# blindopen/TSM-Det-Pointcloud-

Measured on AMD Instinct MI355X. Metric: point-cloud frames/sec (fwd+bwd), higher is better.
Workload: dtype f32; 1 GPU; BASELINE configs[1]: KITTI-shaped synthetic, 20000 pts / 16000 active voxels per frame, full SECOND detector (VoxelBackBone8x) fwd+bwd+AdamW step; batch_per_gpu=4, global_batch=4, parallelism=dp1, voxelize_on_gpu=True

## Files before the change

tsm-det-pointcloud-_amd/csrc/conv_wgrad.hip:

```cpp
#include "spx_common.h"

#ifdef SPX_WG_DIAG
__device__ unsigned long long* g_wg_diag = nullptr;
extern "C" int spx_diag_set(unsigned long long* p) { return (int)hipMemcpyToSymbol(HIP_SYMBOL(g_wg_diag), &p, sizeof(p)); }
#define DIAG_T() __builtin_amdgcn_s_memtime()
#endif

namespace {

typedef float f32x4 __attribute__((ext_vector_type(4)));

#ifndef SPX_SB
#define SPX_SB __builtin_amdgcn_sched_barrier(0)
#endif
constexpr int kGroups = 4;
#ifndef SPX_WG_BURST
#define SPX_WG_BURST 4
#endif
constexpr int kBurst = SPX_WG_BURST;

static inline int wgrad_splits(int64_t n, int cin, int cout, int kvol) {
  int64_t s = n / (64 * kGroups);
  constexpr int slab_mb = 32;
  int64_t by_slab = (int64_t(slab_mb) << 20) / ((int64_t)kvol * cin * cout * 4);
  if (s > by_slab) s = by_slab;
  constexpr int max_blocks = 2048;
  int64_t by_blocks = max_blocks / kvol;
  if (by_blocks < 8) by_blocks = 8;
  if (s > by_blocks) s = by_blocks;
  if (s < 1) s = 1;
  return (int)s;
}

__device__ __forceinline__ void wgrad_plan(const int32_t* __restrict__ cnt, int K, int J, int lane, int& sk, int& start,
                                           int& mycnt) {
  const uint32_t cval = lane < K ? (uint32_t)cnt[lane] : 0u;
  mycnt = (int)cval;
  uint64_t total = cval;
#pragma unroll
  for (int o = 32; o > 0; o >>= 1) total += __shfl_xor(total, o);
  int sh = 0;
  while ((total >> sh) >= (1u << 19)) ++sh;
  const uint32_t tot_s = (uint32_t)(total >> sh);
  sk = 0;
  if (lane < K) sk = tot_s > 0 ? 1 + (int)(((uint32_t)(J - K) * (cval >> sh)) / tot_s) : J / K;
  int incl = sk;
#pragma unroll
  for (int o = 1; o < 64; o <<= 1) {
    int t = __shfl_up(incl, o);
    if (lane >= o) incl += t;
  }
  start = incl - sk;
}

constexpr int kCntUnroll = 4;
__global__ __launch_bounds__(1024) void k_wgrad_count(const int32_t* __restrict__ pair, int64_t ld, int64_t n,
                                                      const int64_t* d_n, int K, int G, int32_t* __restrict__ cnt64,
                                                      int32_t* __restrict__ cnt8) {
  __shared__ int32_t part[16];
  const int x = blockIdx.x, k = blockIdx.y;
  const int lane = threadIdx.x & 63, w = threadIdx.x >> 6;
  const int64_t nlive = spx_live_n(d_n, n);
  const int64_t n8 = ((nlive + 7) / 8 + 63) / 64 * 64;
  const int64_t g0 = x * (n8 / 64);
  int64_t g1 = g0 + n8 / 64;
  const int64_t glive = (nlive + 63) / 64;
  if (g1 > glive) g1 = glive;
  const int32_t* prow = pair + (int64_t)k * ld;
  int total = 0;
  for (int64_t g = g0 + w * kCntUnroll; g < g1; g += 16 * kCntUnroll) {
    int32_t id[kCntUnroll];
#pragma unroll
    for (int u = 0; u < kCntUnroll; ++u) {
      const int64_t row = 64 * (g + u) + lane;
      id[u] = (g + u < g1 && row < nlive) ? prow[row] : -1;
    }
#pragma unroll
    for (int u = 0; u < kCntUnroll; ++u) {
      const int c = __popcll(__ballot(id[u] >= 0));
      if (lane == 0 && g + u < g1) cnt64[(size_t)k * G + g + u] = c;
      total += c;
    }
  }
  if (lane == 0) part[w] = total;
  __syncthreads();
  if (threadIdx.x == 0) {
    int t = 0;
#pragma unroll
    for (int i = 0; i < 16; ++i) t += part[i];
    cnt8[x * 32 + k] = t;
  }
}

template <int W>
__device__ __forceinline__ void load_vec(const float* __restrict__ p, float (&v)[W]) {
  if constexpr (W == 1) {
    v[0] = p[0];
  } else if constexpr (W == 2) {
    float2 t = *reinterpret_cast<const float2*>(p);
    v[0] = t.x, v[1] = t.y;
  } else {
#pragma unroll
    for (int i = 0; i < W; i += 4) {
      float4 t = *reinterpret_cast<const float4*>(p + i);
      v[i] = t.x, v[i + 1] = t.y, v[i + 2] = t.z, v[i + 3] = t.w;
    }
  }
}

template <int W>
__device__ __forceinline__ void store_vec(float* __restrict__ p, const float (&v)[W]) {
  if constexpr (W == 1) {
    p[0] = v[0];
  } else if constexpr (W == 2) {
    *reinterpret_cast<float2*>(p) = make_float2(v[0], v[1]);
  } else {
#pragma unroll
    for (int i = 0; i < W; i += 4) *reinterpret_cast<float4*>(p + i) = make_float4(v[i], v[i + 1], v[i + 2], v[i + 3]);
  }
}

template <int MI, int NJ, bool EXACT, bool FULL>
__device__ __forceinline__ void wgrad_fetch(const float* __restrict__ in, int cin, const float* __restrict__ dout,
                                            int cout, const int32_t* q_src, const int32_t* q_dst, int p, int npairs,
                                            int c, float (&a)[MI], float (&b)[NJ]) {
  const bool has = FULL || (p < npairs);
  const int32_t sid = has ? q_src[p] : 0;
  const int32_t did = has ? q_dst[p] : 0;
  if (EXACT && FULL) {
    load_vec<MI>(in + (size_t)sid * cin + MI * c, a);
    load_vec<NJ>(dout + (size_t)did * cout + NJ * c, b);
  } else {
#pragma unroll
    for (int mi = 0; mi < MI; ++mi) {
      int ci = MI * c + mi;
      a[mi] = (has && ci < cin) ? in[(size_t)sid * cin + ci] : 0.f;
    }
#pragma unroll
    for (int nj = 0; nj < NJ; ++nj) {
      int co = NJ * c + nj;
      b[nj] = (has && co < cout) ? dout[(size_t)did * cout + co] : 0.f;
    }
  }
}

template <int MI, int NJ>
__device__ __forceinline__ void wgrad_mfma_step(f32x4 (&acc)[MI][NJ], const float (&a)[MI], const float (&b)[NJ]) {
#pragma unroll
  for (int mi = 0; mi < MI; ++mi)
#pragma unroll
    for (int nj = 0; nj < NJ; ++nj) acc[mi][nj] = __builtin_amdgcn_mfma_f32_16x16x4f32(a[mi], b[nj], acc[mi][nj], 0, 0, 0);
}

template <int MI, int NJ, bool EXACT>
__global__ __launch_bounds__(64) void k_wgrad_mfma(const float* __restrict__ in, int cin,
                                                   const float* __restrict__ dout, int cout,
                                                   const int32_t* __restrict__ pair, int64_t ld, int64_t n,
                                                   const int64_t* d_n, const int32_t* __restrict__ cnt64,
                                                   const int32_t* __restrict__ cnt8, int G, int J, int K,
                                                   float* __restrict__ slab) {
  __shared__ int32_t q_src[64 * kGroups + 4];
  __shared__ int32_t q_dst[64 * kGroups + 4];
  const int lane = threadIdx.x;
  const int c = lane & 15, q = lane >> 4;
  const int xcd = blockIdx.x & 7, j = blockIdx.x >> 3;
  int sk, start, mycnt;
  wgrad_plan(cnt8 + xcd * 32, K, J, lane, sk, start, mycnt);
  const unsigned long long mine = __ballot(lane < K && j >= start && j < start + sk);
  if (mine == 0) return;
  const int k = __ffsll((long long)mine) - 1;
  const int sub = __builtin_amdgcn_readfirstlane(j - __shfl(start, k));
  const int nsub = __builtin_amdgcn_readfirstlane(__shfl(sk, k));
  const int64_t total = __builtin_amdgcn_readfirstlane(__shfl(mycnt, k));
  const int64_t nlive = spx_live_n(d_n, n);
  const int64_t n8 = ((nlive + 7) / 8 + 63) / 64 * 64;
  const int64_t lo = total * sub / nsub, hi = total * (sub + 1) / nsub;
  const int gx0 = (int)(xcd * (n8 / 64));
  int gx1 = gx0 + (int)(n8 / 64);
  const int glive = (int)((nlive + 63) / 64);
  if (gx1 > glive) gx1 = glive;
  int n_lo = 0, n_hi = 0;
  int64_t run = 0;
  for (int g = gx0; g < gx1; g += 64) {
    const int v = g + lane < gx1 ? cnt64[(size_t)k * G + g + lane] : 0;
    int incl = v;
#pragma unroll
    for (int o = 1; o < 64; o <<= 1) {
      int t = __shfl_up(incl, o);
      if (lane >= o) incl += t;
    }
    const int64_t excl = run + incl - v;
    const bool in = g + lane < gx1;
    n_lo += __popcll(__ballot(in && excl < lo));
    n_hi += __popcll(__ballot(in && excl < hi));
    run += __shfl(incl, 63);
  }
  int64_t r0 = 64 * (int64_t)(gx0 + n_lo);
  int64_t r1 = 64 * (int64_t)(gx0 + n_hi);
  if (r1 > nlive) r1 = nlive;
  if (r0 > r1) r0 = r1;

#ifdef SPX_WG_DIAG
  const unsigned long long d_t0 = DIAG_T(), d_r0 = __builtin_amdgcn_s_memrealtime();
  unsigned long long d_steps = 0, d_loop = 0, d_nsteps = 0;
#endif
  f32x4 acc[MI][NJ];
#pragma unroll
  for (int mi = 0; mi < MI; ++mi)
#pragma unroll
    for (int nj = 0; nj < NJ; ++nj) acc[mi][nj] = f32x4{0.f, 0.f, 0.f, 0.f};

  const int32_t* prow = pair + (int64_t)k * ld;
  int carry = 0;
  int32_t idn[kGroups];
  const int64_t rlast = r1 > r0 ? r1 - 1 : 0;
#pragma unroll
  for (int g = 0; g < kGroups; ++g) {
    int64_t row = r0 + 64 * g + lane;
    idn[g] = prow[row < rlast ? row : rlast];
  }
  for (int64_t base = r0; base < r1; base += 64 * kGroups) {
    int32_t id[kGroups];
#pragma unroll
    for (int g = 0; g < kGroups; ++g) {
      id[g] = base + 64 * g + lane < r1 ? idn[g] : -1;
      int64_t row = base + 64 * (kGroups + g) + lane;
      idn[g] = prow[row < rlast ? row : rlast];
    }
    int nvalid = carry;
#pragma unroll
    for (int g = 0; g < kGroups; ++g) {
      unsigned long long mask = __ballot(id[g] >= 0);
      int rank = nvalid + __builtin_amdgcn_mbcnt_hi((unsigned)(mask >> 32), __builtin_amdgcn_mbcnt_lo((unsigned)mask, 0u));
      if (id[g] >= 0) {
        q_src[rank] = id[g];
        q_dst[rank] = (int32_t)(base + 64 * g + lane);
      }
      nvalid += __popcll(mask);
    }
    const int full = nvalid >> 2;
    carry = nvalid & 3;
    if (full == 0) continue;
    __builtin_amdgcn_wave_barrier();
    const int last = full - 1;
#ifdef SPX_WG_DIAG
    const unsigned long long d_a = DIAG_T();
    d_nsteps += full;
#endif
    for (int st = 0; st < full; st += kBurst) {
      float a[kBurst][MI], b[kBurst][NJ];
#pragma unroll
      for (int g = 0; g < kBurst; ++g) {
        const int sg = st + g < last ? st + g : last;
        wgrad_fetch<MI, NJ, EXACT, true>(in, cin, dout, cout, q_src, q_dst, 4 * sg + q, 4, c, a[g], b[g]);
      }
      asm volatile("" ::: "memory");
      __builtin_amdgcn_sched_barrier(0);
#pragma unroll
      for (int g = 0; g < kBurst; ++g) {
        if (g > 0) {
          const float keep = st + g < full ? 1.f : 0.f;
#pragma unroll
          for (int nj = 0; nj < NJ; ++nj) b[g][nj] *= keep;
        }
        wgrad_mfma_step<MI, NJ>(acc, a[g], b[g]);
      }
    }
#ifdef SPX_WG_DIAG
    d_loop += DIAG_T() - d_a;
#endif
    __builtin_amdgcn_wave_barrier();
    if (carry) {
      int32_t ts = 0, td = 0;
      if (lane < carry) ts = q_src[4 * full + lane], td = q_dst[4 * full + lane];
      __builtin_amdgcn_wave_barrier();
      if (lane < carry) q_src[lane] = ts, q_dst[lane] = td;
    }
    __builtin_amdgcn_wave_barrier();
  }
  int ntail = carry ? 1 : 0;
  ntail = __builtin_amdgcn_readfirstlane(ntail);
  asm volatile("" : "+s"(ntail));
  for (int t = 0; t < ntail; ++t) {
    __builtin_amdgcn_wave_barrier();
    float a0[MI], b0[NJ];
    wgrad_fetch<MI, NJ, EXACT, false>(in, cin, dout, cout, q_src, q_dst, q, carry, c, a0, b0);
    wgrad_mfma_step<MI, NJ>(acc, a0, b0);
  }

#ifdef SPX_WG_DIAG
  if (g_wg_diag && lane == 0) {
    unsigned long long* o = g_wg_diag + (size_t)blockIdx.x * 8;
    const unsigned long long t1 = DIAG_T();
    o[0] = t1 - d_t0;
    o[1] = d_loop;
    o[2] = d_nsteps;
    o[3] = __builtin_amdgcn_s_memrealtime() - d_r0;
    o[4] = k;
    o[5] = d_t0;
    o[6] = t1;
    o[7] = (unsigned long long)(r1 > r0 ? r1 - r0 : 0);
  }
#endif
  float* out = slab + ((size_t)xcd * J + j) * cin * cout;
#pragma unroll
  for (int mi = 0; mi < MI; ++mi)
#pragma unroll
    for (int e = 0; e < 4; ++e) {
      const int ci = MI * (4 * q + e) + mi;
      if (EXACT) {
        float v[NJ];
#pragma unroll
        for (int nj = 0; nj < NJ; ++nj) v[nj] = acc[mi][nj][e];
        store_vec<NJ>(out + (size_t)ci * cout + NJ * c, v);
      } else if (ci < cin) {
#pragma unroll
        for (int nj = 0; nj < NJ; ++nj) {
          int co = NJ * c + nj;
          if (co < cout) out[(size_t)ci * cout + co] = acc[mi][nj][e];
        }
      }
    }
}

constexpr int kRedSlices = 16;
__global__ __launch_bounds__(64 * kRedSlices) void k_wgrad_reduce(const float* __restrict__ slab,
                                                                   const int32_t* __restrict__ cnt8, int J, int K, int cin,
                                                                   int cout, float* __restrict__ dw) {
  __shared__ float part[kRedSlices][64];
  __shared__ int p_off[9][32], p_start[8][32];
  {
    const int w = threadIdx.x >> 6, lane = threadIdx.x & 63;
    if (w < 8) {
      int sk, start, mycnt;
      wgrad_plan(cnt8 + w * 32, K, J, lane, sk, start, mycnt);
      if (lane < 32) p_off[w + 1][lane] = sk, p_start[w][lane] = start;
    }
  }
  __syncthreads();
  if (threadIdx.x < 32) {
    int run = 0;
    for (int x = 0; x < 8; ++x) {
      int v = p_off[x + 1][threadIdx.x];
      p_off[x][threadIdx.x] = run;
      run += v;
    }
    p_off[8][threadIdx.x] = run;
  }
  __syncthreads();
  const int per = cin * cout;
  const int total = K * per;
  const int e = threadIdx.x & 63, sl = threadIdx.x >> 6;
  const int t = blockIdx.x * 64 + e;
  float acc4[4] = {0.f, 0.f, 0.f, 0.f};
  if (t < total) {
    const int k = t / per, el = t - k * per;
    const int len = p_off[8][k];
    int x = 0;
    for (int i = sl; i < len; i += 4 * kRedSlices) {
#pragma unroll
      for (int u = 0; u < 4; ++u) {
        const int ii = i + u * kRedSlices;
        if (ii < len) {
          while (ii >= p_off[x + 1][k]) ++x;
          acc4[u] += slab[((size_t)x * J + p_start[x][k] + (ii - p_off[x][k])) * per + el];
        }
      }
    }
  }
  part[sl][e] = (acc4[0] + acc4[1]) + (acc4[2] + acc4[3]);
  __syncthreads();
  if (sl == 0 && t < total) {
    float v = 0.f;
#pragma unroll
    for (int i = 0; i < kRedSlices; ++i) v += part[i][e];
    int co = t % cout, ci = (t / cout) % cin, k = t / per;
    dw[((size_t)co * K + k) * cin + ci] = v;
  }
}

}

static inline int wgrad_blocks_per_xcd(int64_t n, int cin, int cout, int kvol) {
  int J = (wgrad_splits(n, cin, cout, kvol) * kvol + 7) / 8;
  return J < kvol ? kvol : J;
}

static inline size_t wgrad_slab_bytes(int cin, int cout, int kvol, int64_t n) {
  return spx_align((size_t)8 * wgrad_blocks_per_xcd(n, cin, cout, kvol) * cin * cout * sizeof(float));
}
static inline size_t wgrad_cnt64_bytes(int kvol, int64_t n) {
  return spx_align((size_t)kvol * (size_t)((n + 63) / 64 + 1) * sizeof(int32_t));
}

extern "C" size_t spx_conv_wgrad_ws_bytes(int cin, int cout, int kvol, int64_t n_out) {
  return wgrad_slab_bytes(cin, cout, kvol, n_out) + wgrad_cnt64_bytes(kvol, n_out) + spx_align(8 * 32 * sizeof(int32_t));
}

#define SPX_WG_CASE(A, B)                                                                                          \
  if (MI == A && NJ == B) {                                                                                        \
    if (exact)                                                                                                     \
      hipLaunchKernelGGL((k_wgrad_mfma<A, B, true>), dim3(8 * J), dim3(64), 0, s, in, cin, dout, cout, pair, pair_ld, n_out, \
                         d_n_out, cnt64, cnt8, G, J, kvol, slab);                                                  \
    else                                                                                                           \
      hipLaunchKernelGGL((k_wgrad_mfma<A, B, false>), dim3(8 * J), dim3(64), 0, s, in, cin, dout, cout, pair, pair_ld, n_out, \
                         d_n_out, cnt64, cnt8, G, J, kvol, slab);                                                  \
    launched = true;                                                                                               \
  }

extern "C" size_t spx_conv_wgrad_counts_bytes(int kvol, int64_t n_out) {
  return wgrad_cnt64_bytes(kvol, n_out < 0 ? 0 : n_out) + spx_align(8 * 32 * sizeof(int32_t));
}

extern "C" int spx_conv_wgrad_counts(const int32_t* pair, int64_t pair_ld, int kvol, int64_t n_out, const int64_t* d_n_out,
                                     int32_t* counts, spx_stream_t stream) {
  if (!pair || !counts || kvol <= 0 || kvol > SPX_MAX_KVOL || n_out <= 0 || pair_ld < n_out) return SPX_ERR_INVALID_ARG;
  if (n_out >= (int64_t(1) << 31)) return SPX_ERR_TOO_LARGE;
  const int G = (int)((n_out + 63) / 64 + 1);
  int32_t* cnt8 = reinterpret_cast<int32_t*>(reinterpret_cast<char*>(counts) + wgrad_cnt64_bytes(kvol, n_out));
  hipLaunchKernelGGL(k_wgrad_count, dim3(8, kvol), dim3(1024), 0, spx_s(stream), pair, pair_ld, n_out, d_n_out, kvol, G,
                     counts, cnt8);
  SPX_CHECK_LAUNCH();
  return SPX_OK;
}

extern "C" int spx_conv_wgrad(const float* in, int cin, const float* dout, int cout, int kvol, const int32_t* pair,
                              int64_t pair_ld, int64_t n_out, const int64_t* d_n_out, const int32_t* counts, float* dw,
                              void* ws, size_t ws_bytes, spx_stream_t stream) {
  if (!in || !dout || !pair || !dw || cin <= 0 || cout <= 0 || kvol <= 0 || kvol > SPX_MAX_KVOL || n_out < 0 ||
      pair_ld < n_out)
    return SPX_ERR_INVALID_ARG;
  if (cin > 128 || cout > 128) return SPX_ERR_UNSUPPORTED;
  if (n_out >= (int64_t(1) << 31)) return SPX_ERR_TOO_LARGE;
  if (!ws || ws_bytes < spx_conv_wgrad_ws_bytes(cin, cout, kvol, n_out)) return SPX_ERR_WORKSPACE;
  hipStream_t s = spx_s(stream);
  if (n_out == 0) {
    spx_fill_async(dw, 0, sizeof(float) * (size_t)cout * kvol * cin, s);
    return SPX_OK;
  }
  const int J = wgrad_blocks_per_xcd(n_out, cin, cout, kvol);
  const int G = (int)((n_out + 63) / 64 + 1);
  const int32_t* cnt64 = counts;
  const int32_t* cnt8 = counts ? reinterpret_cast<const int32_t*>(reinterpret_cast<const char*>(counts) + wgrad_cnt64_bytes(kvol, n_out))
                               : nullptr;
  if (!counts) {
    int32_t* c64 = reinterpret_cast<int32_t*>(reinterpret_cast<char*>(ws) + wgrad_slab_bytes(cin, cout, kvol, n_out));
    int32_t* c8 = reinterpret_cast<int32_t*>(reinterpret_cast<char*>(c64) + wgrad_cnt64_bytes(kvol, n_out));
    hipLaunchKernelGGL(k_wgrad_count, dim3(8, kvol), dim3(1024), 0, s, pair, pair_ld, n_out, d_n_out, kvol, G, c64, c8);
    cnt64 = c64;
    cnt8 = c8;
  }
  float* slab = reinterpret_cast<float*>(ws);
  int MI = (cin + 15) / 16, NJ = (cout + 15) / 16;
  if (MI == 3) MI = 4;
  if (MI > 4) MI = 8;
  if (NJ == 3) NJ = 4;
  if (NJ > 4) NJ = 8;
  bool launched = false;
  const bool exact = cin == 16 * MI && cout == 16 * NJ;
  SPX_WG_CASE(1, 1)
  SPX_WG_CASE(1, 2)
  SPX_WG_CASE(1, 4)
  SPX_WG_CASE(1, 8)
  SPX_WG_CASE(2, 1)
  SPX_WG_CASE(2, 2)
  SPX_WG_CASE(2, 4)
  SPX_WG_CASE(2, 8)
  SPX_WG_CASE(4, 1)
  SPX_WG_CASE(4, 2)
  SPX_WG_CASE(4, 4)
  SPX_WG_CASE(4, 8)
  SPX_WG_CASE(8, 1)
  SPX_WG_CASE(8, 2)
  SPX_WG_CASE(8, 4)
  SPX_WG_CASE(8, 8)
  if (!launched) return SPX_ERR_UNSUPPORTED;
  int total = kvol * cin * cout;
  hipLaunchKernelGGL(k_wgrad_reduce, dim3((total + 63) / 64), dim3(64 * kRedSlices), 0, s, slab, cnt8, J, kvol, cin, cout, dw);
  SPX_CHECK_LAUNCH();
  return SPX_OK;
}
```

Before: 295.6 frames/s.

## Team four wgrad waves per block and combine partials in LDS before slab write

The sparse-conv weight-gradient kernel now groups four split waves into one 256-thread block. Waves that work on the same kernel offset add their MFMA accumulators through shared memory, so only the leading wave writes a partial tile to the slab. The slab shrinks from one entry per split to one per run, and the reduce kernel changes to fewer slices with run-based indexing and 32-bit addressing. This cuts slab write and read traffic but adds block barriers, more shared memory per block, and idle waves in teams that straddle offsets.

```diff
diff --git a/tsm-det-pointcloud-_amd/csrc/conv_wgrad.hip b/tsm-det-pointcloud-_amd/csrc/conv_wgrad.hip
--- a/tsm-det-pointcloud-_amd/csrc/conv_wgrad.hip
+++ b/tsm-det-pointcloud-_amd/csrc/conv_wgrad.hip
@@ -51,6 +51,19 @@
     if (lane >= o) incl += t;
   }
   start = incl - sk;
+}
+
+constexpr int kTeam = 4;
+__device__ __forceinline__ void wgrad_runs(int sk, int start, int K, int lane, int& nrun, int& rbase) {
+  nrun = lane < K ? ((start + sk - 1) / kTeam) - (start / kTeam) + 1 : 0;
+  const unsigned long long split = __ballot(lane >= 1 && lane < K && (start % kTeam) != 0);
+  rbase = (start + kTeam - 1) / kTeam +
+          (int)__builtin_amdgcn_mbcnt_hi((unsigned)(split >> 32), __builtin_amdgcn_mbcnt_lo((unsigned)split, 0u));
+}
+
+__host__ __device__ static inline int wgrad_runs_per_xcd(int J, int K) {
+  const int r = (J + kTeam - 1) / kTeam + K - 1;
+  return r < J ? r : J;
 }
 
 constexpr int kCntUnroll = 4;
@@ -152,26 +165,47 @@
     for (int nj = 0; nj < NJ; ++nj) acc[mi][nj] = __builtin_amdgcn_mfma_f32_16x16x4f32(a[mi], b[nj], acc[mi][nj], 0, 0, 0);
 }
 
+template <int MI, int NJ>
+struct WgCombine {
+  static constexpr int kTiles = MI * NJ >= 16 ? 8 : MI * NJ >= 8 ? 4 : MI * NJ >= 2 ? 2 : 1;
+  static constexpr int kPasses = MI * NJ / kTiles;
+};
+
 template <int MI, int NJ, bool EXACT>
-__global__ __launch_bounds__(64) void k_wgrad_mfma(const float* __restrict__ in, int cin,
-                                                   const float* __restrict__ dout, int cout,
-                                                   const int32_t* __restrict__ pair, int64_t ld, int64_t n,
-                                                   const int64_t* d_n, const int32_t* __restrict__ cnt64,
-                                                   const int32_t* __restrict__ cnt8, int G, int J, int K,
-                                                   float* __restrict__ slab) {
-  __shared__ int32_t q_src[64 * kGroups + 4];
-  __shared__ int32_t q_dst[64 * kGroups + 4];
-  const int lane = threadIdx.x;
+__global__ __launch_bounds__(64 * kTeam) void k_wgrad_mfma(const float* __restrict__ in, int cin,
+                                                           const float* __restrict__ dout, int cout,
+                                                           const int32_t* __restrict__ pair, int64_t ld, int64_t n,
+                                                           const int64_t* d_n, const int32_t* __restrict__ cnt64,
+                                                           const int32_t* __restrict__ cnt8, int G, int J, int K,
+                                                           float* __restrict__ slab) {
+  constexpr int kTiles = WgCombine<MI, NJ>::kTiles, kPasses = WgCombine<MI, NJ>::kPasses;
+  __shared__ int32_t q_src_all[kTeam][64 * kGroups + 4];
+  __shared__ int32_t q_dst_all[kTeam][64 * kGroups + 4];
+  __shared__ f32x4 comb[kTeam - 1][kTiles][64];
+  const int lane = threadIdx.x & 63;
+  const int w = __builtin_amdgcn_readfirstlane((int)(threadIdx.x >> 6));
+  int32_t* const q_src = q_src_all[w];
+  int32_t* const q_dst = q_dst_all[w];
   const int c = lane & 15, q = lane >> 4;
-  const int xcd = blockIdx.x & 7, j = blockIdx.x >> 3;
+  const int xcd = blockIdx.x & 7, team = blockIdx.x >> 3;
+  const int j = kTeam * team + w;
   int sk, start, mycnt;
   wgrad_plan(cnt8 + xcd * 32, K, J, lane, sk, start, mycnt);
+  int nrun, rbase;
+  wgrad_runs(sk, start, K, lane, nrun, rbase);
   const unsigned long long mine = __ballot(lane < K && j >= start && j < start + sk);
-  if (mine == 0) return;
-  const int k = __ffsll((long long)mine) - 1;
-  const int sub = __builtin_amdgcn_readfirstlane(j - __shfl(start, k));
-  const int nsub = __builtin_amdgcn_readfirstlane(__shfl(sk, k));
-  const int64_t total = __builtin_amdgcn_readfirstlane(__shfl(mycnt, k));
+  const bool idle = mine == 0;
+  const int k = idle ? 0 : __ffsll((long long)mine) - 1;
+  const int start_k = __builtin_amdgcn_readfirstlane(__shfl(start, k));
+  const int sub = idle ? 0 : __builtin_amdgcn_readfirstlane(j - start_k);
+  const int nsub = idle ? 1 : __builtin_amdgcn_readfirstlane(__shfl(sk, k));
+  const int64_t total = idle ? 0 : __builtin_amdgcn_readfirstlane(__shfl(mycnt, k));
+  const int w_first = start_k > kTeam * team ? start_k - kTeam * team : 0;
+  const int w_end_ = start_k + nsub - kTeam * team;
+  const int w_end = w_end_ < kTeam ? w_end_ : kTeam;
+  const bool leader = !idle && w == w_first;
+  const bool follower = !idle && w != w_first;
+  const int run_slot = __builtin_amdgcn_readfirstlane(__shfl(rbase, k)) + team - start_k / kTeam;
   const int64_t nlive = spx_live_n(d_n, n);
   const int64_t n8 = ((nlive + 7) / 8 + 63) / 64 * 64;
   const int64_t lo = total * sub / nsub, hi = total * (sub + 1) / nsub;
@@ -289,8 +323,8 @@
   }
 
 #ifdef SPX_WG_DIAG
-  if (g_wg_diag && lane == 0) {
-    unsigned long long* o = g_wg_diag + (size_t)blockIdx.x * 8;
+  if (g_wg_diag && lane == 0 && !idle) {
+    unsigned long long* o = g_wg_diag + ((size_t)blockIdx.x * kTeam + w) * 8;
     const unsigned long long t1 = DIAG_T();
     o[0] = t1 - d_t0;
     o[1] = d_loop;
@@ -302,7 +336,29 @@
     o[7] = (unsigned long long)(r1 > r0 ? r1 - r0 : 0);
   }
 #endif
-  float* out = slab + ((size_t)xcd * J + j) * cin * cout;
+  constexpr int kChunk = kTiles < 4 ? kTiles : 4;
+#pragma unroll
+  for (int ps = 0; ps < kPasses; ++ps) {
+    if (follower) {
+#pragma unroll
+      for (int i = 0; i < kTiles; ++i) comb[w - 1][i][lane] = acc[(ps * kTiles + i) / NJ][(ps * kTiles + i) % NJ];
+    }
+    __syncthreads();
+    if (leader) {
+      for (int f = w + 1; f < w_end; ++f) {
+#pragma unroll
+        for (int i0 = 0; i0 < kTiles; i0 += kChunk) {
+#pragma unroll
+          for (int i = i0; i < i0 + kChunk; ++i)
+            acc[(ps * kTiles + i) / NJ][(ps * kTiles + i) % NJ] += comb[f - 1][i][lane];
+          __builtin_amdgcn_sched_barrier(0);
+        }
+      }
+    }
+    if (ps + 1 < kPasses) __syncthreads();
+  }
+  if (!leader) return;
+  float* out = slab + ((size_t)xcd * wgrad_runs_per_xcd(J, K) + run_slot) * cin * cout;
 #pragma unroll
   for (int mi = 0; mi < MI; ++mi)
 #pragma unroll
@@ -323,18 +379,23 @@
     }
 }
 
-constexpr int kRedSlices = 16;
+constexpr int kRedSlices = 4;
+constexpr int kRedUnroll = 4;
 __global__ __launch_bounds__(64 * kRedSlices) void k_wgrad_reduce(const float* __restrict__ slab,
                                                                    const int32_t* __restrict__ cnt8, int J, int K, int cin,
                                                                    int cout, float* __restrict__ dw) {
   __shared__ float part[kRedSlices][64];
-  __shared__ int p_off[9][32], p_start[8][32];
+  __shared__ int p_off[9][32], p_base[8][32];
   {
-    const int w = threadIdx.x >> 6, lane = threadIdx.x & 63;
-    if (w < 8) {
-      int sk, start, mycnt;
-      wgrad_plan(cnt8 + w * 32, K, J, lane, sk, start, mycnt);
-      if (lane < 32) p_off[w + 1][lane] = sk, p_start[w][lane] = start;
+    const int w = __builtin_amdgcn_readfirstlane((int)(threadIdx.x >> 6));
+#pragma unroll
+    for (int x = w; x < 8; x += kRedSlices) {
+      int lane = threadIdx.x & 63;
+      asm volatile("" : "+v"(lane));
+      int sk, start, mycnt, nrun, rbase;
+      wgrad_plan(cnt8 + x * 32, K, J, lane, sk, start, mycnt);
+      wgrad_runs(sk, start, K, lane, nrun, rbase);
+      if (lane < 32) p_off[x + 1][lane] = nrun, p_base[x][lane] = rbase;
     }
   }
   __syncthreads();
@@ -350,25 +411,38 @@
   __syncthreads();
   const int per = cin * cout;
   const int total = K * per;
+  const int RJ = wgrad_runs_per_xcd(J, K);
   const int e = threadIdx.x & 63, sl = threadIdx.x >> 6;
   const int t = blockIdx.x * 64 + e;
-  float acc4[4] = {0.f, 0.f, 0.f, 0.f};
+  float accu[kRedUnroll];
+#pragma unroll
+  for (int u = 0; u < kRedUnroll; ++u) accu[u] = 0.f;
   if (t < total) {
     const int k = t / per, el = t - k * per;
     const int len = p_off[8][k];
     int x = 0;
-    for (int i = sl; i < len; i += 4 * kRedSlices) {
-#pragma unroll
-      for (int u = 0; u < 4; ++u) {
+    for (int i = sl; i < len; i += kRedUnroll * kRedSlices) {
+      int slot[kRedUnroll];
+#pragma unroll
+      for (int u = 0; u < kRedUnroll; ++u) {
         const int ii = i + u * kRedSlices;
+        slot[u] = -1;
         if (ii < len) {
           while (ii >= p_off[x + 1][k]) ++x;
-          acc4[u] += slab[((size_t)x * J + p_start[x][k] + (ii - p_off[x][k])) * per + el];
+          slot[u] = x * RJ + p_base[x][k] + (ii - p_off[x][k]);
         }
       }
-    }
-  }
-  part[sl][e] = (acc4[0] + acc4[1]) + (acc4[2] + acc4[3]);
+      float v[kRedUnroll];
+#pragma unroll
+      for (int u = 0; u < kRedUnroll; ++u)
+        v[u] = slot[u] >= 0 ? *reinterpret_cast<const float*>(reinterpret_cast<const char*>(slab) +
+                                                               4u * ((uint32_t)slot[u] * (uint32_t)per + (uint32_t)el))
+                            : 0.f;
+#pragma unroll
+      for (int u = 0; u < kRedUnroll; ++u) accu[u] += v[u];
+    }
+  }
+  part[sl][e] = (accu[0] + accu[1]) + (accu[2] + accu[3]);
   __syncthreads();
   if (sl == 0 && t < total) {
     float v = 0.f;
@@ -387,7 +461,7 @@
 }
 
 static inline size_t wgrad_slab_bytes(int cin, int cout, int kvol, int64_t n) {
-  return spx_align((size_t)8 * wgrad_blocks_per_xcd(n, cin, cout, kvol) * cin * cout * sizeof(float));
+  return spx_align((size_t)8 * wgrad_runs_per_xcd(wgrad_blocks_per_xcd(n, cin, cout, kvol), kvol) * cin * cout * sizeof(float));
 }
 static inline size_t wgrad_cnt64_bytes(int kvol, int64_t n) {
   return spx_align((size_t)kvol * (size_t)((n + 63) / 64 + 1) * sizeof(int32_t));
@@ -400,10 +474,10 @@
 #define SPX_WG_CASE(A, B)                                                                                          \
   if (MI == A && NJ == B) {                                                                                        \
     if (exact)                                                                                                     \
-      hipLaunchKernelGGL((k_wgrad_mfma<A, B, true>), dim3(8 * J), dim3(64), 0, s, in, cin, dout, cout, pair, pair_ld, n_out, \
+      hipLaunchKernelGGL((k_wgrad_mfma<A, B, true>), dim3(8 * ((J + kTeam - 1) / kTeam)), dim3(64 * kTeam), 0, s, in, cin, dout, cout, pair, pair_ld, n_out, \
                          d_n_out, cnt64, cnt8, G, J, kvol, slab);                                                  \
     else                                                                                                           \
-      hipLaunchKernelGGL((k_wgrad_mfma<A, B, false>), dim3(8 * J), dim3(64), 0, s, in, cin, dout, cout, pair, pair_ld, n_out, \
+      hipLaunchKernelGGL((k_wgrad_mfma<A, B, false>), dim3(8 * ((J + kTeam - 1) / kTeam)), dim3(64 * kTeam), 0, s, in, cin, dout, cout, pair, pair_ld, n_out, \
                          d_n_out, cnt64, cnt8, G, J, kvol, slab);                                                  \
     launched = true;                                                                                               \
   }
```

Measured after the change: 294.3 frames/s. About the same (-0.5%).
